# daooshee/ReReVST-Code

Hardware: AMD Instinct MI355X
Metric: stylized frames/sec at 512x512, 1 style (higher is better)
Workload: dtype f32

## Files before the change

include/rerevst_hip.h:

```cpp
#ifndef REREVST_HIP_H
#define REREVST_HIP_H

#include <stddef.h>
#include <stdint.h>

#ifdef __cplusplus
extern "C" {
#endif

typedef struct rrv_ctx* rrv_handle;

enum {
    RRV_OK = 0,
    RRV_E_ARG = -1,
    RRV_E_HIP = -2,
    RRV_E_WEIGHTS = -3,
    RRV_E_STATE = -4,
    RRV_E_NOMEM = -5,
    RRV_E_DEBUG = -6,
    RRV_E_COMM = -7
};

#define RRV_STATE_FLOATS 17536
#define RRV_MAX_STYLES 8
// ... 157 lines not shown
int rrv_set_yuv16_matrix(rrv_handle h, const float m[12]);
int rrv_set_yuv16_input_matrix(rrv_handle h, const float n[12]);

int rrv_prepare_style_image_device(rrv_handle h, const void* d_style, rrv_image_desc in, int Hs, int Ws, int style_id, void* hip_stream);
int rrv_add_image_device(rrv_handle h, const void* d_frame, rrv_image_desc in, int H, int W, void* hip_stream);

int rrv_get_preclamp(rrv_handle h, float* out, int H, int W);
int rrv_get_preclamp_image(rrv_handle h, float* out, int H, int W, int b);

int rrv_sync(rrv_handle h);

int rrv_set_pipeline(rrv_handle h, int n_slots);

int rrv_set_grid_share(rrv_handle h, int share);

int rrv_set_host_io(rrv_handle h, int mode);

int rrv_debug_copy_tensor(rrv_handle h, int slot, int index, int H, int W, float* host, size_t cap, size_t* floats);

int rrv_debug_copy_tensor_ex(rrv_handle h, int slot, int index, int image, int H, int W, float* host, size_t cap, size_t* floats,
                             int* layout, int* channels);

#define RRV_DBG_STATE_SET 0
#define RRV_DBG_STYLE_PRED 1
int rrv_debug_copy_state(rrv_handle h, int what, int slot, int image, float* out, int n);

int rrv_set_caller_stream(rrv_handle h, void* hip_stream, int enable);

int rrv_host_alloc(size_t bytes, void** out);
int rrv_host_free(void* p);
// ... 18 lines not shown
```

rerevst-code_amd/_lib.py:

```python
import ctypes as C
import os

HERE = os.path.dirname(os.path.abspath(__file__))
LIB_PATH = os.environ.get("RRV_LIB_PATH") or os.path.join(HERE, "librerevst_hip.so")
STATE_FLOATS = 17536
MAX_STYLES = 8

_lib = None


class ImageDesc(C.Structure):
    _fields_ = [("dtype", C.c_int), ("layout", C.c_int), ("space", C.c_int)]


DT_U8, DT_F32 = 0, 1
DT_U16 = 2
LAY_HWC_BGR, LAY_CHW_RGB = 0, 1
LAY_I420, LAY_NV12 = 2, 3
LAY_I420_16, LAY_P016 = 8, 9
YUV_BT601, YUV_BT709 = 0, 1
SP_PIXEL, SP_UNIT, SP_NORM = 0, 1, 2
TF_PAD_CROP, TF_FRAME_MODE, TF_ON_STREAM, TF_WEIGHTS_DEVICE = 1, 2, 4, 8
DBG_STATE_SET, DBG_STYLE_PRED = 0, 1

# ... 74 lines not shown
    "rrv_yuv_input_matrix_depth": (C.c_int, [C.c_int, C.c_int, C.c_int, C.POINTER(C.c_float)]),
    "rrv_set_yuv16_matrix": (C.c_int, [C.c_void_p, C.POINTER(C.c_float)]),
    "rrv_set_yuv16_input_matrix": (C.c_int, [C.c_void_p, C.POINTER(C.c_float)]),
    "rrv_prepare_style_image_device": (C.c_int, [C.c_void_p, C.c_void_p, ImageDesc, C.c_int, C.c_int, C.c_int, C.c_void_p]),
    "rrv_add_image_device": (C.c_int, [C.c_void_p, C.c_void_p, ImageDesc, C.c_int, C.c_int, C.c_void_p]),
    "rrv_get_preclamp": (C.c_int, [C.c_void_p, C.c_void_p, C.c_int, C.c_int]),
    "rrv_get_preclamp_image": (C.c_int, [C.c_void_p, C.c_void_p, C.c_int, C.c_int, C.c_int]),
    "rrv_sync": (C.c_int, [C.c_void_p]),
    "rrv_set_pipeline": (C.c_int, [C.c_void_p, C.c_int]),
    "rrv_set_host_io": (C.c_int, [C.c_void_p, C.c_int]),
    "rrv_debug_copy_tensor": (C.c_int, [C.c_void_p, C.c_int, C.c_int, C.c_int, C.c_int, C.c_void_p, C.c_size_t, C.POINTER(C.c_size_t)]),
    "rrv_debug_copy_tensor_ex": (C.c_int, [C.c_void_p, C.c_int, C.c_int, C.c_int, C.c_int, C.c_int, C.c_void_p, C.c_size_t,
                                           C.POINTER(C.c_size_t), C.POINTER(C.c_int), C.POINTER(C.c_int)]),
    "rrv_debug_copy_state": (C.c_int, [C.c_void_p, C.c_int, C.c_int, C.c_int, C.c_void_p, C.c_int]),
    "rrv_set_grid_share": (C.c_int, [C.c_void_p, C.c_int]),
    "rrv_set_caller_stream": (C.c_int, [C.c_void_p, C.c_void_p, C.c_int]),
    "rrv_host_alloc": (C.c_int, [C.c_size_t, C.POINTER(C.c_void_p)]),
    "rrv_host_free": (C.c_int, [C.c_void_p]),
    "rrv_host_register": (C.c_int, [C.c_void_p, C.c_size_t]),
    "rrv_host_unregister": (C.c_int, [C.c_void_p]),
    "rrv_set_debug": (C.c_int, [C.c_void_p, C.c_int]),
    "rrv_debug_selftest": (C.c_int, [C.c_void_p]),
    "rrv_debug_fail_alloc": (C.c_int, [C.c_void_p, C.c_int]),
    "rrv_profile_begin": (C.c_int, [C.c_void_p]),
    "rrv_profile_end": (C.c_int, [C.c_void_p]),
    "rrv_profile_count": (C.c_int, [C.c_void_p]),
    "rrv_profile_entry": (C.c_int, [C.c_void_p, C.c_int, C.POINTER(C.c_char_p), C.POINTER(C.c_float),
                                    C.POINTER(C.c_double), C.POINTER(C.c_double), C.POINTER(C.c_double)]),
}

# ... 41 lines not shown
```

rerevst-code_amd/build.py:

```python
import os
import subprocess
import sys

HERE = os.path.dirname(os.path.abspath(__file__))
CSRC = os.path.join(HERE, "csrc")
LIB = os.path.join(HERE, "librerevst_hip.so")
SOURCES = ["rerevst_hip.hip"]
HEADERS = ["conv_mfma.h", "conv_wino.h", "conv_ups5.h", "conv_wino_split.h", "conv_f43.h", "conv_thin.h", "prep_kernels.h", "mask_kernels.h", "../../include/rerevst_hip.h"]


def _stale():
    if not os.path.exists(LIB):
        return True
    t = os.path.getmtime(LIB)
    return any(os.path.getmtime(os.path.join(CSRC, f)) > t for f in SOURCES + HEADERS)


def build_lib(force=False, verbose=True, extra=()):
    if not force and not _stale():
        return LIB
    hipcc = os.environ.get("HIPCC", "/opt/rocm/bin/hipcc")
    cmd = [hipcc, "--offload-arch=gfx950", "-O3", "-std=c++17", "-shared", "-fPIC",
           "-Wno-unused-result", *extra,
           *[os.path.join(CSRC, s) for s in SOURCES], "-o", LIB]
# ... 9 lines not shown
```

rerevst-code_amd/csrc/conv_mfma.h:

```cpp
#pragma once
#include <hip/hip_runtime.h>
#include <stdint.h>

typedef float f32x16 __attribute__((ext_vector_type(16)));
typedef float f32x4 __attribute__((ext_vector_type(4)));

enum {
    E_RELU = 1,
    E_LRELU = 2,
    E_NORM1 = 4,
    E_RES = 8,
    E_RES_UPS = 16,
    E_NORM2 = 32,
    E_POOL = 64
};

struct ConvP {
    const float* in;
    int Hi, Wi, Cin;
    float* out;
    int H, W, Cout;
    int B;
    int in_bstride0;
    const float* wpk;
    const float* bias;
    const float* n1;
    const float* res;
    int Hr, Wr;
    const float* n2;
    const float* sty;
    int tiles_x, tiles_y;
    int xcd_slabs;
    float* sc_out;
    int ty0, tx0;
    long long* dbg;
    int cstride;
    int cin_slab_step;
    int par_bstride, bias_bstride;
    long long w_bstride;
    int out_p8;
};

template <int BN>
struct WaveCfg {
    static constexpr int WAVES_N = (BN >= 64) ? 2 : 1;
    static constexpr int WAVES_M = 4 / WAVES_N;
    static constexpr int WN_SUB = BN / 32 / WAVES_N;
    static constexpr int WM_SUB = 4 / WAVES_M;
};

__device__ __forceinline__ void glds16(const float* src, char* lds_wave_base) {
    __builtin_amdgcn_global_load_lds((const __attribute__((address_space(1))) void*)src,
                                     (__attribute__((address_space(3))) void*)lds_wave_base, 16, 0, 0);
}
// ... 244 lines not shown
```

rerevst-code_amd/csrc/rerevst_hip.hip:

```cpp
#include <hip/hip_runtime.h>
#include <dlfcn.h>
#include <stddef.h>
#include <stdint.h>
#include <string.h>
#include <algorithm>
#include <cmath>
#include <thread>
#include <stdio.h>
#include <map>
#include <condition_variable>
#include <mutex>
#include <string>
#include <vector>

#include "../../include/rerevst_hip.h"
#include "conv_mfma.h"
#include "conv_wino.h"
#include "conv_wino_split.h"
#include "conv_f43.h"
#include "conv_thin.h"
#include "prep_kernels.h"
#include "mask_kernels.h"

namespace {

const int NORM_CH[11] = {512, 512, 256, 128, 64, 256, 256, 128, 128, 64, 64};
enum { N_DEC0 = 0, N_DEC1, N_DEC2, N_DEC3, N_DEC4, N_S4N1, N_S4N2, N_S3N1, N_S3N2, N_S2N1, N_S2N2 };
const int STYLE_CH[4] = {64, 128, 256, 512};
struct StateLayout {
    int norm[11], filt[6], sty[4];
    StateLayout() {
        int o = 0;
        for (int i = 0; i < 11; ++i) { norm[i] = o; o += 4 * NORM_CH[i]; }
// ... 162 lines not shown
    PrepPlan prep;
    uint8_t* pend_u8 = nullptr; size_t pend_cap = 0; int pend_n = 0;
    InFmt pend_in = IN_BGR8;
    static constexpr int BLEND_W_RING = 4, BLEND_W_FLOATS = 64 * RRV_MAX_STYLES;
    struct BlendW { float* dev = nullptr; float* pin = nullptr; hipEvent_t ev[BLEND_W_RING] = {nullptr}; bool used[BLEND_W_RING] = {false}; unsigned gen = 0; } blend_w[2];
    const float* last_pre = nullptr; int last_pre_H = 0, last_pre_W = 0, last_pre_B = 0;
    struct StageBufs { uint8_t* in = nullptr; void* out = nullptr; size_t in_cap = 0, out_cap = 0; };
    struct HostStage {
        StageBufs dev, pin; hipEvent_t in_done = nullptr, k_done = nullptr, out_done = nullptr;
        float *mask = nullptr, *mask_pin = nullptr; size_t mask_cap = 0, mask_pin_cap = 0;
    } hstage[4];
    hipStream_t copy_in = nullptr, copy_out = nullptr;
    struct Ticket { long id = -1; void* out = nullptr; size_t out_bytes = 0; bool open = false; } tickets[4];
    long next_ticket = 0;
    int grid_share = 1;
    int f43_mode = 1;
    unsigned f43_layers = F43_DEFAULT_LAYERS;
    bool illcond = false;
    bool enc_p8_tables = false;
    int p8 = 3;
    bool f43_path = false;
    unsigned direct_layers = 0;
    int ms_group = 0;
    YuvSide yuv_in, yuv_out;
    int host_io = 0;
    int n_cus = 256;
    int debug = 0;
    int fail_alloc_in = 0;
    bool profiling = false;
    std::vector<ProfEntry> prof;
// ... 182 lines not shown
    return RRV_OK;
}

struct ConvCall {
    const Tens* in; Tens* out; const ConvW* w;
    int H, W;
    bool ups = false; int epi = 0;
    Tens* sc_out = nullptr;
    int wy0 = 0, wx0 = 0, wy1 = 0, wx1 = 0;
    const float* n1 = nullptr; const Tens* res = nullptr; const float* n2 = nullptr; const float* sty = nullptr;
    int B = 1;
    int ksplit = 0;
    const float* bias = nullptr;
    int par_bstride = 0, bias_bstride = 0; long long w_bstride = 0;
    bool direct = false;
    bool in_p8 = false, out_p8 = false;
};

template <int BN, int TAPS, int EPI>
void conv_launch(const ConvP& p, dim3 grid, hipStream_t s) {
    hipLaunchKernelGGL((conv_mfma_k<BN, TAPS, EPI>), grid, dim3(256), 0, s, p);
}

typedef void (*ConvFn)(const ConvP&, dim3, hipStream_t);
typedef hipError_t (*AttrFn)();
struct ConvKey { int BN, TAPS, UPS, EPI; ConvFn fn; const char* name; AttrFn attr; ConvFn fn_img = nullptr; };
#define CK(BN, TAPS, UPS, EPI) {BN, TAPS, UPS, EPI, &conv_launch<BN, TAPS, EPI>, "conv_mfma<" #BN "," #TAPS "," #EPI ">", nullptr}
const ConvKey CONV_TABLE[] = {
    CK(128, 1, 0, 0), CK(64, 1, 0, 0),
    CK(32, 9, 0, 0),
// ... 11 lines not shown
}
template <int EPI, int NW, int UPS, int SC, int PERIMG = 0>
hipError_t wino_attr() {
    hipError_t e = hipFuncSetAttribute((const void*)conv_wino_k<EPI, 0, NW, UPS, SC, 0>, hipFuncAttributeMaxDynamicSharedMemorySize, wino_smem<NW, UPS, SC>());
    if (e == hipSuccess && PERIMG) e = hipFuncSetAttribute((const void*)conv_wino_k<EPI, 0, NW, UPS, SC, 1>, hipFuncAttributeMaxDynamicSharedMemorySize, wino_smem<NW, UPS, SC>());
    return e;
}
template <int EPI, int PERIMG>
void wsplit_launch(const ConvP& p, dim3 grid, hipStream_t s) {
    hipLaunchKernelGGL((conv_wino_split_k<EPI, PERIMG>), grid, dim3(512), WSPLIT_SMEM_BYTES, s, p);
}
template <int EPI, int PERIMG>
hipError_t wsplit_attr() {
    hipError_t e = hipFuncSetAttribute((const void*)conv_wino_split_k<EPI, 0>, hipFuncAttributeMaxDynamicSharedMemorySize, WSPLIT_SMEM_BYTES);
    if (e == hipSuccess && PERIMG) e = hipFuncSetAttribute((const void*)conv_wino_split_k<EPI, 1>, hipFuncAttributeMaxDynamicSharedMemorySize, WSPLIT_SMEM_BYTES);
    return e;
}
template <int EPI, int LAY = 0>
void f43_launch(const ConvP& p, dim3 grid, hipStream_t s) {
    hipLaunchKernelGGL((conv_f43_k<EPI, LAY>), grid, dim3(F43Geo::NT), F43Geo::SMEM, s, p);
}
template <int EPI, int LAY = 0>
hipError_t f43_attr() { return hipFuncSetAttribute((const void*)conv_f43_k<EPI, LAY>, hipFuncAttributeMaxDynamicSharedMemorySize, F43Geo::SMEM); }
#define FK(EPI) {32, 9, 0, EPI, &f43_launch<EPI>, "conv_f43<" #EPI ">", &f43_attr<EPI>, nullptr}
struct F43LayKey { int EPI, LAY; ConvFn fn; const char* name; AttrFn attr; };
#define FKL(EPI, LAY) {EPI, LAY, &f43_launch<EPI, LAY>, "conv_f43<" #EPI ", " #LAY ">", &f43_attr<EPI, LAY>}
#define WK(EPI) {32, 9, 0, EPI, &wsplit_launch<EPI, 0>, "conv_wino<" #EPI ">", &wsplit_attr<EPI, 0>, nullptr}
#define WKI(EPI) {32, 9, 0, EPI, &wsplit_launch<EPI, 0>, "conv_wino<" #EPI ">", &wsplit_attr<EPI, 1>, &wsplit_launch<EPI, 1>}
#define UW(EPI) {32, 9, 1, EPI, &wino_launch<EPI, UPW_NW, 1, 0>, "conv_upw<" #EPI ">", &wino_attr<EPI, UPW_NW, 1, 0>}
#define UWS(EPI) {32, 29, 1, EPI, &wino_launch<EPI, UPW_NW, 1, 1>, "conv_upw_sc<" #EPI ">", &wino_attr<EPI, UPW_NW, 1, 1>}
#define UWSI(EPI) {32, 29, 1, EPI, &wino_launch<EPI, UPW_NW, 1, 1>, "conv_upw_sc<" #EPI ">", &wino_attr<EPI, UPW_NW, 1, 1, 1>, &wino_launch<EPI, UPW_NW, 1, 1, 1>}
const ConvKey WINO_TABLE[] = {
    WK(E_RELU), WK(E_RELU | E_POOL), WKI(E_RELU | E_NORM1) , WKI(E_LRELU | E_NORM1 | E_RES_UPS | E_NORM2), WKI(E_LRELU),
    WKI(0),
    WKI(E_RES), WKI(E_RES | E_NORM2),
    UW(E_LRELU | E_NORM1), UW(E_LRELU),
    UWSI(E_LRELU | E_NORM1),
    UWS(E_LRELU),
};

const ConvKey F43_TABLE[] = { FK(E_RELU), FK(E_RELU | E_POOL), FK(E_RELU | E_NORM1), FK(E_LRELU | E_NORM1 | E_RES_UPS | E_NORM2) };
const F43LayKey F43_LAY_TABLE[] = {
    FKL(E_RELU | E_POOL, 3), FKL(E_RELU, 3),
    FKL(E_RELU | E_POOL, 1),
    FKL(E_LRELU | E_NORM1 | E_RES_UPS | E_NORM2, 1),
};

unsigned resident_wgs(rrv_handle h, int occ) {
    unsigned r = (unsigned)h->n_cus * (unsigned)occ;
    if (h->grid_share > 1) {
        r = (r / h->grid_share) & ~7u;
        if (r < 8) r = 8;
    }
    return r;
}
// ... 19 lines not shown
    const ConvKey* k = nullptr;
    bool wino = false;
    bool f43 = !c.direct && use_f43(h, w, c.B, c.H, c.W, c.epi, c.ups, c.ksplit, c.bias_bstride != 0 || c.w_bstride != 0) &&
               !((c.wy0 | c.wx0 | c.wy1 | c.wx1) & 31);
    if (f43) {
        f43 = false;
        for (const ConvKey& e : F43_TABLE)
            if (e.EPI == c.epi) { k = &e; f43 = true; wino = true; break; }
    }
    const bool fuse_sc = c.ups && c.sc_out != nullptr;
    if (fuse_sc && !w.pk_ups_sc) return fail(h, RRV_E_ARG, "conv: no shortcut-fused pack for this layer");
    if (!f43 && !c.direct && (c.ups ? w.pk_ups != nullptr : w.pk_wino != nullptr)) {
        for (const ConvKey& e : WINO_TABLE)
            if (e.EPI == c.epi && e.UPS == (int)c.ups && (e.TAPS == 29) == fuse_sc) { k = &e; wino = true; break; }
    }
    const int ks = c.ksplit > 1 ? c.ksplit : 1;
    if (ks > 1 && !(wino && !c.ups && w.Cout == 32 && (w.Cin % (32 * ks)) == 0 && c.bias))
        return fail(h, RRV_E_ARG, "conv: split K needs the row-split kernel, a 32-cout layer, an even number of 16-channel chunks per slice and a split bias");
    if (!k && !c.ups) {
        for (const ConvKey& e : CONV_TABLE)
            if (e.BN == w.BN && e.TAPS == w.taps && e.EPI == c.epi) { k = &e; break; }
    }
    if (!k) {
        char b[128];
        snprintf(b, sizeof b, "no conv kernel for BN=%d taps=%d ups=%d epi=%d", w.BN, w.taps, (int)c.ups, c.epi);
        return fail(h, RRV_E_ARG, b);
    }
    const int lay = (c.in_p8 ? 1 : 0) | (c.out_p8 ? 2 : 0);
    ConvFn lay_fn = nullptr;
    const char* lay_name = nullptr;
// ... 10 lines not shown
    p.in_bstride0 = 1;
    p.wpk = f43 ? w.pk_f43 : wino ? (c.ups ? (fuse_sc ? w.pk_ups_sc : w.pk_ups) : w.pk_wino) : w.pk; p.bias = w.bias;
    if (fuse_sc) {
        if (c.sc_out->H != c.in->H || c.sc_out->W != c.in->W || c.sc_out->C != w.Cout) return fail(h, RRV_E_ARG, "conv: shortcut output geometry mismatch");
        p.sc_out = c.sc_out->p;
    }
    if (!p.wpk) return fail(h, RRV_E_ARG, "conv: weights not packed for this kernel"); p.n1 = c.n1; p.n2 = c.n2; p.sty = c.sty;
    if (c.bias) p.bias = c.bias;
    p.par_bstride = c.par_bstride; p.bias_bstride = c.bias_bstride; p.w_bstride = c.w_bstride;
    if (ups_p8) { if (!wino) return fail(h, RRV_E_ARG, "conv: no upsample-fused kernel for this layer"); p.out_p8 = 1; }
    if ((c.par_bstride | c.bias_bstride || c.w_bstride) && !wino) return fail(h, RRV_E_ARG, "conv: per-image state needs a transform-domain kernel");
    if (c.ups && (c.bias_bstride || c.w_bstride)) return fail(h, RRV_E_ARG, "conv: the upsample-fused kernel shares weights and bias over the images of a launch");
    if (ks > 1) {
        p.Cin = w.Cin / ks; p.cstride = w.Cin; p.cin_slab_step = w.Cin / ks; p.Cout = 32 * ks;
    }
    if (c.res) { p.res = c.res->p; p.Hr = c.res->H; p.Wr = c.res->W; }
    p.tiles_x = (c.W + 15) / 16; p.tiles_y = (c.H + 7) / 8;
    if ((c.in_p8 ? c.in->C != 8 || c.in->B < c.B * (w.Cin / 8) : c.in->C != w.Cin) ||
        (c.out_p8 ? c.out->C != 8 || c.out->B < c.B * (w.Cout / 8) : c.out->C != w.Cout * ks)) return fail(h, RRV_E_ARG, "conv: channel mismatch");
    const int eh = c.ups ? c.H / 2 : c.H, ew = c.ups ? c.W / 2 : c.W;
    if (c.in->H != eh || c.in->W != ew + (c.in_p8 ? 6 : 0)) return fail(h, RRV_E_ARG, "conv: input geometry mismatch");
    const int oh = (c.epi & E_POOL) ? c.H / 2 : c.H, ow = (c.epi & E_POOL) ? c.W / 2 : c.W;
    if (c.out->H != oh || c.out->W != ow + (c.out_p8 ? 6 : 0)) return fail(h, RRV_E_ARG, "conv: output geometry mismatch");
    const int TS = f43 || fuse_sc ? 32 : 16;
    if (wino) { p.tiles_x = (c.W + TS - 1) / TS; p.tiles_y = (c.H + TS - 1) / TS; }
    double win_frac = 1.0;
    if (wino && c.wy1 > c.wy0 && c.wx1 > c.wx0) {
        if ((c.wy0 | c.wx0 | c.wy1 | c.wx1) & 15) return fail(h, RRV_E_ARG, "conv: window must be tile aligned");
        int wy0 = c.wy0, wx0 = c.wx0, wy1 = c.wy1, wx1 = c.wx1;
        if (TS == 32 && !f43) {
            wy0 &= ~31; wx0 &= ~31; wy1 = (wy1 + 31) & ~31; wx1 = (wx1 + 31) & ~31;
            if (wy1 > ((c.H + 31) & ~31)) wy1 = (c.H + 31) & ~31;
            if (wx1 > ((c.W + 31) & ~31)) wx1 = (c.W + 31) & ~31;
        }
        p.ty0 = wy0 / TS; p.tx0 = wx0 / TS;
        p.tiles_y = (wy1 - wy0) / TS; p.tiles_x = (wx1 - wx0) / TS;
        const int TD = fuse_sc ? 32 : 16;
        win_frac = ((double)(wy1 - wy0) * (wx1 - wx0)) / ((double)((c.H + TD - 1) / TD * TD) * ((c.W + TD - 1) / TD * TD));
    }
    dim3 grid((unsigned)(p.tiles_x * p.tiles_y * c.B), (unsigned)(w.Cout / w.BN));
    if (wino) {
        const unsigned slabs = (unsigned)(w.Cout / 32) * ks;
        const unsigned items = (unsigned)(p.tiles_x * p.tiles_y * c.B) * slabs;
        const unsigned resident = resident_wgs(h, fuse_sc ? Ups5Geo::OCC : c.ups ? WinoGeo<UPW_NW, 1>::OCC : 1);
        grid = dim3(items < resident ? items : resident, 1);
        p.xcd_slabs = (grid.x % 8 == 0 && (grid.x / 8) % slabs == 0) ? 1 : 0;
    }
    const double px = (double)c.B * c.H * c.W * win_frac;
    const double cin = w.Cin;
    const double flops_sc = fuse_sc ? 2.0 * c.B * c.in->H * c.in->W * (double)w.Cout * cin : 0.0;
    const double flops = 2.0 * px * w.Cout * cin * w.taps + flops_sc;
    const double flops_exec = 2.0 * px * w.Cout * cin * (f43 ? 2.25 : wino ? (c.ups ? (fuse_sc ? 29.0 / 16.0 : 2.25) : 4.0) : (double)w.taps);
    const double bytes = 4.0 * ((double)c.B * c.in->H * c.in->W * cin + (double)c.B * oh * ow * w.Cout +
                                (c.res ? (double)c.B * c.res->H * c.res->W * w.Cout : 0.0) + (double)w.Cout * cin * w.taps +
                                (fuse_sc ? (double)c.B * c.in->H * c.in->W * w.Cout + (double)w.Cout * cin : 0.0));
    hipStream_t s = h->stream;
    ConvFn fn = lay_fn ? lay_fn : k->fn;
    if (wino && !f43 && (c.par_bstride | c.bias_bstride || c.w_bstride)) {
        if (!k->fn_img) return fail(h, RRV_E_ARG, "conv: this layer has no per-image-state kernel");
        fn = k->fn_img;
    }
    stamp(h, c.out, c.B);
    if (fuse_sc) stamp(h, c.sc_out, c.B);
    if (h->profiling) {
        char nm[160];
        snprintf(nm, sizeof nm, "%s@%dx%d@%dx%d", lay_name ? lay_name : k->name, w.Cin, w.Cout, c.H, c.W);
        return launch(h, nm, flops, bytes, [&] { fn(p, grid, s); }, flops_exec);
    }
    return launch(h, lay_name ? lay_name : k->name, flops, bytes, [&] { fn(p, grid, s); }, flops_exec);
// ... 387 lines not shown
    d.B = B; d.H = H; d.W = W;
    return RRV_OK;
}

int filter_down(rrv_handle h, const Tens* cur, DecPlan& d, int f, int B) {
    const int split = kf_split(cur->H, cur->W);
    if (split == 1) {
        ConvCall c{cur, &d.d, &h->cur->fold_down[f], cur->H, cur->W}; c.B = B; c.epi = E_LRELU;
        if (h->state_images) { c.w_bstride = 32 * 512 * 16; c.bias_bstride = 256; }
        return conv(h, c);
    }
    Tens& t = d.dpart;
    ConvCall c{cur, &t, &h->cur->fold_down[f], cur->H, cur->W}; c.B = B; c.epi = 0; c.ksplit = split; c.bias = h->cur->fold_down[f].bias;
    if (h->state_images) { c.w_bstride = 32 * 512 * 16; c.bias_bstride = 256; }
    RCHK(conv(h, c));
    const long npix = (long)B * (d.d.H + 2) * (d.d.W + 2);
    stamp(h, &d.d, B);
    return launch(h, "sum_parts", 0, 4.0 * 32 * (split + 1) * npix, [&] {
        const long nb = (npix * 8 + 255) / 256;
        hipLaunchKernelGGL(sum_parts_lrelu_k, dim3((unsigned)(nb < 4096 ? nb : 4096)), dim3(256), 0, h->stream, (const float*)t.p, d.d.p, split, npix);
    });
}

int filter_up(rrv_handle h, const Tens* cur, DecPlan& d, Tens* out, int f, int B) {
    const float* st = h->cur->active;
    ConvCall u{&d.d, out, &h->cur->fold_up[f], cur->H, cur->W}; u.B = B;
    if (h->state_images) { u.w_bstride = 512 * 32 * 16; u.par_bstride = RRV_STATE_FLOATS; }
    u.epi = E_RES | (f == 2 ? E_NORM2 : 0); u.res = cur;
    if (f == 2) { u.n2 = st + SL.norm[N_DEC1]; u.sty = st + SL.sty[3]; }
    return conv(h, u);
}

struct Win { int y0, x0, y1, x1; };

struct BlkDesc { const char* name; int cout, n1, n2, nada, sty; };
const BlkDesc BLKS[3] = {{"slice4", 256, N_S4N1, N_S4N2, N_DEC2, 2}, {"slice3", 128, N_S3N1, N_S3N2, N_DEC3, 1}, {"slice2", 64, N_S2N1, N_S2N2, N_DEC4, 0}};

int resblock_frame(rrv_handle h, int B, int k, const Tens& in, DecPlan& d, const Win* wa = nullptr, const Win* wo = nullptr) {
    const BlkDesc& b = BLKS[k];
    Tens &xs = d.xs[k], &a = d.a[k], &o = d.o[k], &qa = d.qa[k];
    const float* st = h->cur->active;
// ... 556 lines not shown
    h->dev = device;
    (void)rrv_yuv_input_matrix(RRV_YUV_BT601, 0, h->yuv_in.m8);
    (void)rrv_yuv_matrix(RRV_YUV_BT601, 0, h->yuv_out.m8);
    bool ok = hipSetDevice(device) == hipSuccess;
    for (int i = 0; ok && i < RRV_MAX_SLOTS; ++i) ok = hipStreamCreateWithFlags(&h->streams[i], hipStreamNonBlocking) == hipSuccess;
    if (!ok) {
        delete h;
        return RRV_E_HIP;
    }
    h->stream = h->streams[0];
    ok = ok && hipStreamCreateWithFlags(&h->copy_in, hipStreamNonBlocking) == hipSuccess && hipStreamCreateWithFlags(&h->copy_out, hipStreamNonBlocking) == hipSuccess;
    for (int i = 0; ok && i < RRV_MAX_SLOTS; ++i) ok = hipEventCreateWithFlags(&h->slot_ev[i], hipEventDisableTiming) == hipSuccess;
    for (auto& st : h->hstage)
        for (hipEvent_t* e : {&st.in_done, &st.k_done, &st.out_done}) ok = ok && hipEventCreateWithFlags(e, hipEventDisableTiming) == hipSuccess;
    for (const ConvKey& e : WINO_TABLE)
        if (ok && e.attr) ok = e.attr() == hipSuccess;
    for (const ConvKey& e : F43_TABLE)
        if (ok && e.attr) ok = e.attr() == hipSuccess;
    for (const F43LayKey& e : F43_LAY_TABLE)
        if (ok && e.attr) ok = e.attr() == hipSuccess;
    if (!ok) {
        delete h;
        return RRV_E_HIP;
    }
    {
        hipDeviceProp_t prop;
        if (hipGetDeviceProperties(&prop, device) == hipSuccess && prop.multiProcessorCount > 0) h->n_cus = prop.multiProcessorCount;
        const int masked = cu_mask_count(getenv("HSA_CU_MASK"), device, h->n_cus);
        if (masked > 0 && masked < h->n_cus) h->n_cus = masked;
        if (const char* e = getenv("RRV_CUS")) { const int n = atoi(e); if (n >= 1 && n <= 1024) h->n_cus = n; }
// ... 1568 lines not shown
int rrv_sync(rrv_handle h) {
    if (!h) return RRV_E_ARG;
    HIPCHK(hipSetDevice(h->dev));
    return sync_all(h);
}

int rrv_set_pipeline(rrv_handle h, int n_slots) {
    if (!h || n_slots < 1 || n_slots > RRV_MAX_SLOTS) return RRV_E_ARG;
    HIPCHK(hipSetDevice(h->dev));
    RCHK(sync_all(h));
    h->n_slots = n_slots;
    h->next_slot = 0;
    return RRV_OK;
}

int rrv_set_grid_share(rrv_handle h, int share) {
    if (!h || share < 1 || share > 4) return RRV_E_ARG;
    h->grid_share = share;
    return RRV_OK;
}

int rrv_set_f43(rrv_handle h, int mode) {
    if (!h || mode < 0 || mode > 2) return RRV_E_ARG;
    RCHK(sync_all(h));
    h->f43_mode = mode;
    return RRV_OK;
}

int rrv_set_multistyle_group(rrv_handle h, int frames) {
    if (!h || frames < 0 || frames > rrv_ctx::MS_GROUP_MAX) return RRV_E_ARG;
// ... 159 lines not shown
```

rerevst-code_amd/framework.py:

```python
import collections
import ctypes as C

import numpy as np

from . import _lib
from .video import YUV_FORMATS, YUV_FORMAT_NAMES, YUV_STANDARDS, _yuv_depth, yuv_frame_bytes
from .weights import weight_table, load_checkpoint


class RRVError(RuntimeError):
    pass


def pinned_empty(shape, dtype=np.float32):
    import weakref
    lib = _lib.load()
    dt = np.dtype(dtype)
    n = int(np.prod(shape)) * dt.itemsize
    ptr = C.c_void_p()
    if lib.rrv_host_alloc(max(n, 1), C.byref(ptr)) != 0:
        raise MemoryError("rrv_host_alloc(%d) failed" % n)
    buf = (C.c_char * max(n, 1)).from_address(ptr.value)
    weakref.finalize(buf, lib.rrv_host_free, ptr)
    return np.frombuffer(buf, dtype=dt, count=int(np.prod(shape))).reshape(shape)
# ... 597 lines not shown
                    a.out_desc, flags | (_lib.TF_WEIGHTS_DEVICE if wd is not None else 0), stream))
                continue
            self._chk(plain_fn(self._h, C.c_void_p(xb[b0].data_ptr()), a.in_desc, nb, a.H, a.W,
                               C.c_void_p(ob[b0].data_ptr()), a.out_desc, flags, stream))
        return out

    def sync(self):
        self._chk(self._lib.rrv_sync(self._h))

    def set_caller_stream(self, stream_ptr, enable=True):
        self._chk(self._lib.rrv_set_caller_stream(self._h, C.c_void_p(stream_ptr), 1 if enable else 0))

    def set_f43(self, mode):
        self._chk(self._lib.rrv_set_f43(self._h, int(mode)))

    def set_grid_share(self, share):
        self._chk(self._lib.rrv_set_grid_share(self._h, int(share)))

    def debug_tensor(self, slot, index, H, W):
        n = C.c_size_t(0)
        self._chk(self._lib.rrv_debug_copy_tensor(self._h, int(slot), int(index), int(H), int(W), None, 0, C.byref(n)))
        out = np.empty(n.value, np.float32)
        self._chk(self._lib.rrv_debug_copy_tensor(self._h, int(slot), int(index), int(H), int(W), out.ctypes.data_as(C.c_void_p), n.value, C.byref(n)))
        return out

    def debug_tensor_ex(self, slot, index, H, W, image=0):
        n, lay, ch = C.c_size_t(0), C.c_int(0), C.c_int(0)
        args = (self._h, int(slot), int(index), int(image), int(H), int(W))
        self._chk(self._lib.rrv_debug_copy_tensor_ex(*args, None, 0, C.byref(n), C.byref(lay), C.byref(ch)))
        out = np.empty(n.value, np.float32)
# ... 149 lines not shown
```

Before: 836.2.

## Fuse split-K partial sum and LeakyReLU into KernelFilter up-conv Winograd kernel

Adds a dedicated Winograd up-convolution kernel for the 32-channel KernelFilter path that reads the split-K partial-sum tensor directly, sums the parts and applies LeakyReLU while staging input tiles into LDS. This removes the separate sum_parts_lrelu kernel launch and its write and re-read of the summed tensor. The kernel also walks a contiguous span of (tile, output-slab) units per workgroup, so an input tile is transformed once and reused across output slabs. The cost is reading the wider partial-sum input inside the conv, plus a more complex kernel with hand-placed waits and barriers.

```diff
diff --git a/include/rerevst_hip.h b/include/rerevst_hip.h
--- a/include/rerevst_hip.h
+++ b/include/rerevst_hip.h
@@ -195,6 +195,8 @@
 
 int rrv_set_grid_share(rrv_handle h, int share);
 
+int rrv_set_kf_up(rrv_handle h, int mode);
+
 int rrv_set_host_io(rrv_handle h, int mode);
 
 int rrv_debug_copy_tensor(rrv_handle h, int slot, int index, int H, int W, float* host, size_t cap, size_t* floats);
diff --git a/rerevst-code_amd/_lib.py b/rerevst-code_amd/_lib.py
--- a/rerevst-code_amd/_lib.py
+++ b/rerevst-code_amd/_lib.py
@@ -112,6 +112,7 @@
                                            C.POINTER(C.c_size_t), C.POINTER(C.c_int), C.POINTER(C.c_int)]),
     "rrv_debug_copy_state": (C.c_int, [C.c_void_p, C.c_int, C.c_int, C.c_int, C.c_void_p, C.c_int]),
     "rrv_set_grid_share": (C.c_int, [C.c_void_p, C.c_int]),
+    "rrv_set_kf_up": (C.c_int, [C.c_void_p, C.c_int]),
     "rrv_set_caller_stream": (C.c_int, [C.c_void_p, C.c_void_p, C.c_int]),
     "rrv_host_alloc": (C.c_int, [C.c_size_t, C.POINTER(C.c_void_p)]),
     "rrv_host_free": (C.c_int, [C.c_void_p]),
diff --git a/rerevst-code_amd/build.py b/rerevst-code_amd/build.py
--- a/rerevst-code_amd/build.py
+++ b/rerevst-code_amd/build.py
@@ -6,7 +6,7 @@
 CSRC = os.path.join(HERE, "csrc")
 LIB = os.path.join(HERE, "librerevst_hip.so")
 SOURCES = ["rerevst_hip.hip"]
-HEADERS = ["conv_mfma.h", "conv_wino.h", "conv_ups5.h", "conv_wino_split.h", "conv_f43.h", "conv_thin.h", "prep_kernels.h", "mask_kernels.h", "../../include/rerevst_hip.h"]
+HEADERS = ["conv_mfma.h", "conv_wino.h", "conv_ups5.h", "conv_wino_split.h", "conv_wino_up32.h", "conv_f43.h", "conv_thin.h", "prep_kernels.h", "mask_kernels.h", "../../include/rerevst_hip.h"]
 
 
 def _stale():
diff --git a/rerevst-code_amd/csrc/conv_mfma.h b/rerevst-code_amd/csrc/conv_mfma.h
--- a/rerevst-code_amd/csrc/conv_mfma.h
+++ b/rerevst-code_amd/csrc/conv_mfma.h
@@ -38,6 +38,8 @@
     int cin_slab_step;
     int par_bstride, bias_bstride;
     long long w_bstride;
+    int in_parts;
+    int slab_span;
     int out_p8;
 };
 
diff --git a/rerevst-code_amd/csrc/conv_wino_up32.h b/rerevst-code_amd/csrc/conv_wino_up32.h
--- /dev/null
+++ b/rerevst-code_amd/csrc/conv_wino_up32.h
@@ -0,0 +1,262 @@
+#pragma once
+#include "conv_wino_split.h"
+
+#ifndef WUP32_ABL
+#define WUP32_ABL 0
+#endif
+#define WUP32_STAGE_GROUP 3
+
+#define WUP32_SMEM_BYTES (WSPLIT_SMEM_BYTES + WINO_PAR_BYTES)
+
+template <int EPI, int PERIMG = 0>
+__global__ __launch_bounds__(512, 1) void conv_wino_up32_k(const ConvP p) {
+    static_assert((EPI & ~(E_RES | E_NORM2)) == 0 && (EPI & E_RES), "the KernelFilter up-convolution: residual, optional second normalisation");
+    using G = WinoGeo<8, 0>;
+    constexpr int RAW_BYTES = G::RAW_BYTES, U_BYTES = G::U_BYTES, U_LDS = G::U_LDS, NT = G::NT;
+    static_assert(G::U_IT == 4, "U block = 4 LDS-DMA instructions per thread");
+    extern __shared__ __attribute__((aligned(16))) char smem[];
+    const int tid = threadIdx.x;
+    const int wave = __builtin_amdgcn_readfirstlane(tid >> 6);
+    const int lane = tid & 63, t = lane & 15, q = lane >> 4;
+    const int tr = t >> 3, tc = t & 7;
+    const int tg = wave >> 1;
+    const int half = wave & 1;
+    const float sgn = half ? -1.f : 1.f;
+    const int cs = p.cstride;
+    const int n_ntiles = p.Cout >> 5;
+
+    const int n_units = p.tiles_x * p.tiles_y * p.B * n_ntiles;
+    int unit = blockIdx.x * p.slab_span;
+    const int unit_end = min(unit + p.slab_span, n_units);
+    struct Item { int tx, ty, b, s0, s1; };
+    auto item_at = [&](int u) {
+        Item r;
+        const int pix = u / n_ntiles;
+        r.s0 = u - pix * n_ntiles;
+        r.s1 = min(n_ntiles, r.s0 + unit_end - u);
+        r.tx = pix % p.tiles_x; r.ty = (pix / p.tiles_x) % p.tiles_y; r.b = pix / (p.tiles_x * p.tiles_y);
+        return r;
+    };
+    auto in_of = [&](const Item& a) {
+        return p.in + (size_t)a.b * (size_t)(p.Hi + 2) * (p.Wi + 2) * cs + (size_t)(((a.ty + p.ty0) * 16) * (p.Wi + 2) + (a.tx + p.tx0) * 16) * cs;
+    };
+    auto w_of = [&](const Item& a) { return p.wpk + (size_t)a.s0 * (2 * 16 * 32 * 16) + (PERIMG ? (size_t)a.b * p.w_bstride : (size_t)0); };
+
+    char* const par = smem + 2 * RAW_BYTES + 2 * U_LDS;
+    char* const xch = par + 2 * WINO_PAR_BYTES;
+    auto stage_params = [&](int ntile, int img) {
+        if (wave < 2) {
+            const int e = tid;
+            const int row = e >> 3, col = (e & 7) * 4;
+            const float* src = p.bias;
+            const int pb = PERIMG ? img * p.par_bstride : 0;
+            int off = ntile * 32 + col + (PERIMG ? img * p.bias_bstride : 0);
+            if (row >= 5 && row <= 8) { src = (EPI & E_NORM2) ? p.n2 : p.bias; off = (EPI & E_NORM2) ? ntile * 32 + col + pb + (row - 5) * p.Cout : off; }
+            if (row >= 9) { src = (EPI & E_NORM2) ? p.sty : p.bias; off = (EPI & E_NORM2) ? ntile * 32 + col + pb + (row - 9) * p.Cout : off; }
+            if (row > 10) { src = p.bias; off = ntile * 32 + (PERIMG ? img * p.bias_bstride : 0); }
+            glds16(src + off, par + (ntile & 1) * WINO_PAR_BYTES + wave * 1024);
+        }
+    };
+
+    constexpr int N_PIECE = 324 * 8, N_ROWS = (N_PIECE + NT - 1) / NT;
+    struct Piece { int src, dst; };
+    auto piece_at = [&](int row) {
+        const int e = row * NT + tid;
+        const bool ok = e < N_PIECE;
+        const int P = ok ? e >> 3 : 0, cq = ok ? e & 7 : 0;
+        const int hf = P >= G::HALF, rem = P - hf * G::HALF;
+        const int hy = rem / 9, hx = 2 * (rem - hy * 9) + hf;
+        return Piece{(hy * (p.Wi + 2) + hx) * cs + 4 * cq, ok ? (cq >> 2) * RAW_BYTES + P * 64 + (((cq & 3) ^ ((hx >> 1) & 3)) << 4) : -1};
+    };
+    auto piece_load = [&](const float* in_t, const Piece pc, auto& part) {
+        constexpr int PARTS = sizeof(part) / sizeof(part[0]);
+#pragma unroll
+        for (int k = 0; k < PARTS; ++k) part[k] = *(const f32x4*)(in_t + pc.src + 32 * k);
+    };
+    auto piece_store = [&](const Piece pc, const auto& part) {
+        constexpr int PARTS = sizeof(part) / sizeof(part[0]);
+        f32x4 o = part[0];
+#pragma unroll
+        for (int k = 1; k < PARTS; ++k) o += part[k];
+        if (PARTS > 1) {
+#pragma unroll
+            for (int c = 0; c < 4; ++c) o[c] = o[c] >= 0.f ? o[c] : o[c] * 0.2f;
+        }
+        if (pc.dst >= 0) *(f32x4*)(smem + pc.dst) = o;
+    };
+
+    const unsigned lds0 = (unsigned)(size_t)(__attribute__((address_space(3))) char*)smem;
+    const unsigned offU = lds0 + 2 * RAW_BYTES + t * 64 + ((q ^ ((0 - (t >> 2)) & 3)) << 4);
+    const unsigned ubA = offU + (half ? 12 : 0) * 2048;
+    const unsigned ubB = offU + (half ? 8 : 4) * 2048;
+
+    f32x4 acc[8][2];
+    f32x4 va[8], vb[8];
+    auto transform = [&](int chunk, f32x4 (&v)[8]) {
+        f32x4 d[12];
+#pragma unroll
+        for (int dx = 0; dx < 4; ++dx)
+#pragma unroll
+            for (int b = 0; b < 3; ++b) {
+                const int hy = 4 * tg + 2 * tr + (half ? 3 - b : b), hx = 2 * tc + dx;
+                const int P = (hx & 1) * G::HALF + hy * 9 + (hx >> 1);
+                d[dx * 3 + b] = *(const f32x4*)(smem + chunk * RAW_BYTES + P * 64 + ((q ^ ((hx >> 1) & 3)) << 4));
+            }
+#pragma unroll
+        for (int dx = 0; dx < 4; ++dx) {
+            v[dx * 2 + 0] = f4sub(d[dx * 3 + 0], d[dx * 3 + 2]);
+            v[dx * 2 + 1] = f4fma(d[dx * 3 + 2], sgn, d[dx * 3 + 1]);
+        }
+#pragma unroll
+        for (int rl = 0; rl < 2; ++rl) {
+            const f32x4 e0 = v[0 + rl], e1 = v[2 + rl], e2 = v[4 + rl], e3 = v[6 + rl];
+            v[0 + rl] = f4sub(e0, e2); v[2 + rl] = f4add(e1, e2); v[4 + rl] = f4sub(e2, e1); v[6 + rl] = f4sub(e1, e3);
+        }
+    };
+
+    auto chunk_body = [&](auto par_c, const f32x4 (&vcur)[8], const rsrc_t rs_u, const int usoff, auto&& hook) {
+        constexpr int PAR = decltype(par_c)::value;
+        constexpr bool FIRST = PAR == 0;
+        char* const udst = smem + 2 * RAW_BYTES + (1 - PAR) * U_LDS;
+        constexpr int UI = PAR * U_LDS;
+        f32x4 u[4][2];
+        u[0][0] = lds_rd128<UI + 0>(ubA); u[0][1] = lds_rd128<UI + 1024>(ubA);
+        u[1][0] = lds_rd128<UI + 2048>(ubA); u[1][1] = lds_rd128<UI + 2048 + 1024>(ubA);
+        static_for([&](auto ic) {
+            constexpr int i = decltype(ic)::value;
+            if constexpr (i + 2 < 8) {
+                constexpr int n = i + 2, k = n & 3;
+                u[n & 3][0] = lds_rd128<UI + k * 2048>(n < 4 ? ubA : ubB);
+                u[n & 3][1] = lds_rd128<UI + k * 2048 + 1024>(n < 4 ? ubA : ubB);
+            }
+            lds_release2<(i + 1 < 8 ? 2 : 0) + (i + 2 < 8 ? 2 : 0)>(u[i & 3][0], u[i & 3][1]);
+            __builtin_amdgcn_sched_barrier(0);
+            if constexpr (i < G::U_IT) bufld16_rs(rs_u, udst + (i * NT + wave * 64) * 16, tid * 16, usoff + i * NT * 16);
+            const f32x4 vv = vcur[(i & 3) * 2 + (i >> 2)];
+#pragma unroll
+            for (int s = 0; s < 4; ++s)
+#pragma unroll
+                for (int nb = 0; nb < 2; ++nb)
+                    acc[i][nb] = __builtin_amdgcn_mfma_f32_16x16x4f32(u[i & 3][nb][s], vv[s], (FIRST && s == 0) ? f32x4{0.f, 0.f, 0.f, 0.f} : acc[i][nb], 0, 0, 0);
+            hook(ic);
+        }, std::make_integer_sequence<int, 8>{});
+    };
+    auto no_hook = [](auto) {};
+
+    auto run = [&](auto parts_c) {
+        constexpr int PARTS = decltype(parts_c)::value;
+        Item cur{};
+        bool have = unit < unit_end;
+        const float* w_t = p.wpk;
+        const float* in_t = p.in;
+        if (have) {
+            cur = item_at(unit);
+            w_t = w_of(cur);
+            in_t = in_of(cur);
+#pragma unroll
+            for (int it = 0; it < G::U_IT; ++it) bufld16(w_t, smem + 2 * RAW_BYTES + (it * NT + wave * 64) * 16, tid * 16, it * NT * 16);
+        }
+        while (have) {
+            if (!(WUP32_ABL & 1) || unit == (int)blockIdx.x * p.slab_span) {
+                for (int g = 0; g < N_ROWS; g += WUP32_STAGE_GROUP) {
+                    f32x4 part[WUP32_STAGE_GROUP][PARTS];
+#pragma unroll
+                    for (int j = 0; j < WUP32_STAGE_GROUP; ++j) if (g + j < N_ROWS) piece_load(in_t, piece_at(g + j), part[j]);
+#pragma unroll
+                    for (int j = 0; j < WUP32_STAGE_GROUP; ++j) if (g + j < N_ROWS) piece_store(piece_at(g + j), part[j]);
+                }
+            }
+            __syncthreads();
+            transform(0, va);
+            transform(1, vb);
+            const int e_y0 = (cur.ty + p.ty0) * 16, e_x0 = (cur.tx + p.tx0) * 16, e_b = cur.b;
+            const int n_slabs = cur.s1 - cur.s0;
+            unit += n_slabs;
+            const bool have_nxt = unit < unit_end;
+            Item nxt = cur;
+            if (have_nxt) nxt = item_at(unit);
+            const float* w_n = have_nxt ? w_of(nxt) : w_t;
+            const float* in_n = have_nxt ? in_of(nxt) : in_t;
+            const rsrc_t rs_t = make_rsrc(w_t), rs_n = make_rsrc(w_n);
+            const float* res_b = p.res + (size_t)e_b * (size_t)(p.Hr + 2) * (p.Wr + 2) * p.Cout;
+            const int yb = e_y0 + 4 * tg + 2 * tr, xb = e_x0 + 2 * tc;
+            const int y = yb + half;
+            int rpix[2];
+#pragma unroll
+            for (int j = 0; j < 2; ++j) rpix[j] = (y < p.H && xb + j < p.W) ? ((y + 1) * (p.Wr + 2) + xb + j + 1) * p.Cout : 0;
+
+            const rsrc_t rs_out = make_rsrc(p.out + (size_t)e_b * (size_t)(p.H + 2) * (p.W + 2) * p.Cout);
+            constexpr unsigned NO_PIXEL = 0x80000000u;
+            unsigned pend_off[2] = {NO_PIXEL, NO_PIXEL};
+            int pend_par = 0;
+            f32x4 Tc[2][2];
+            f32x4 resv[2][2];
+            const char* const theirs = xch + (wave ^ 1) * 4096 + lane * 16;
+            auto epi_step = [&](auto ic) {
+                constexpr int nb = decltype(ic)::value >> 1, j = decltype(ic)::value & 1;
+                const char* pl = par + pend_par * WINO_PAR_BYTES + (nb * 16 + 4 * q) * 4;
+                const f32x4 bias = *(const f32x4*)(pl);
+                const f32x4 rc = *(const f32x4*)(theirs + (j * 2 + nb) * 1024);
+                const f32x4 Y = e4add(Tc[j][nb], rc);
+                f32x4 o = e4add(Y, bias);
+                o = e4add(o, resv[nb][j]);
+                if (EPI & E_NORM2) {
+                    const f32x4 m2 = *(const f32x4*)(pl + 640), r2 = *(const f32x4*)(pl + 768), lo2 = *(const f32x4*)(pl + 896), hi2 = *(const f32x4*)(pl + 1024);
+                    const f32x4 smean = *(const f32x4*)(pl + 1152), sstd = *(const f32x4*)(pl + 1280);
+                    o = e4fma(f4norm_clamp(o, m2, r2, lo2, hi2), sstd, smean);
+                }
+#if defined(__HIP_DEVICE_COMPILE__)
+                typedef unsigned u32x4 __attribute__((ext_vector_type(4)));
+                if constexpr (!(WUP32_ABL & 2)) __builtin_amdgcn_raw_buffer_store_b128(__builtin_bit_cast(u32x4, o), rs_out, (int)(pend_off[j] + nb * 64), 0, 0);
+#endif
+            };
+            constexpr int N_ST = (WUP32_ABL & 2) ? 0 : 1;
+
+            for (int r = 0; r < n_slabs; ++r) {
+                const int e_ntile = cur.s0 + r;
+                stage_params(e_ntile, e_b);
+                auto hook0 = [&](auto ic) {
+                    if constexpr (decltype(ic)::value < 4) epi_step(ic);
+                    if constexpr (decltype(ic)::value == 4) {
+#pragma unroll
+                        for (int nb = 0; nb < 2; ++nb)
+#pragma unroll
+                            for (int j = 0; j < 2; ++j) resv[nb][j] = *(const f32x4*)(res_b + rpix[j] + e_ntile * 32 + 4 * q + nb * 16);
+                    }
+                };
+                const bool last = r + 1 == n_slabs;
+                chunk_body(std::integral_constant<int, 0>{}, va, rs_t, (2 * r + 1) * U_BYTES, hook0);
+                if constexpr (!(WUP32_ABL & 4)) asm volatile("s_waitcnt vmcnt(%0) lgkmcnt(0)\n\ts_barrier" :: "n"(4 + N_ST) : "memory");
+                chunk_body(std::integral_constant<int, 1>{}, vb, last ? rs_n : rs_t, last ? 0 : (2 * r + 2) * U_BYTES, no_hook);
+                asm volatile("s_nop 15\n\ts_nop 15\n\ts_nop 15" : "+v"(acc[0][0]), "+v"(acc[0][1]), "+v"(acc[1][0]), "+v"(acc[1][1]), "+v"(acc[2][0]), "+v"(acc[2][1]), "+v"(acc[3][0]), "+v"(acc[3][1]), "+v"(acc[4][0]), "+v"(acc[4][1]), "+v"(acc[5][0]), "+v"(acc[5][1]), "+v"(acc[6][0]), "+v"(acc[6][1]), "+v"(acc[7][0]), "+v"(acc[7][1]));
+                char* mine = xch + wave * 4096 + lane * 16;
+#pragma unroll
+                for (int nb = 0; nb < 2; ++nb) {
+                    f32x4 T[2][2];
+#pragma unroll
+                    for (int rl = 0; rl < 2; ++rl) {
+                        T[rl][0] = e4add(e4add(acc[rl * 4 + 0][nb], acc[rl * 4 + 1][nb]), acc[rl * 4 + 2][nb]);
+                        T[rl][1] = f4sub(f4sub(acc[rl * 4 + 1][nb], acc[rl * 4 + 2][nb]), acc[rl * 4 + 3][nb]);
+                    }
+#pragma unroll
+                    for (int j = 0; j < 2; ++j) {
+                        *(f32x4*)(mine + (j * 2 + nb) * 1024) = T[1][j];
+                        Tc[j][nb] = f4fma(T[1][j], sgn, T[0][j]);
+                    }
+                }
+                if constexpr (!(WUP32_ABL & 4)) __syncthreads();
+#pragma unroll
+                for (int j = 0; j < 2; ++j)
+                    pend_off[j] = (y < p.H && xb + j < p.W) ? (unsigned)((((y + 1) * (p.W + 2) + xb + j + 1) * p.Cout + e_ntile * 32 + 4 * q) * 4) : NO_PIXEL;
+                pend_par = e_ntile & 1;
+            }
+            static_for([&](auto ic) { epi_step(ic); }, std::make_integer_sequence<int, 4>{});
+            cur = nxt; have = have_nxt; w_t = w_n; in_t = in_n;
+        }
+    };
+    if (p.in_parts == 8) run(std::integral_constant<int, 8>{});
+    else if (p.in_parts == 4) run(std::integral_constant<int, 4>{});
+    else if (p.in_parts == 2) run(std::integral_constant<int, 2>{});
+    else run(std::integral_constant<int, 1>{});
+    asm volatile("s_waitcnt vmcnt(0)" ::: "memory");
+}
diff --git a/rerevst-code_amd/csrc/rerevst_hip.hip b/rerevst-code_amd/csrc/rerevst_hip.hip
--- a/rerevst-code_amd/csrc/rerevst_hip.hip
+++ b/rerevst-code_amd/csrc/rerevst_hip.hip
@@ -17,6 +17,7 @@
 #include "conv_mfma.h"
 #include "conv_wino.h"
 #include "conv_wino_split.h"
+#include "conv_wino_up32.h"
 #include "conv_f43.h"
 #include "conv_thin.h"
 #include "prep_kernels.h"
@@ -209,6 +210,7 @@
     struct Ticket { long id = -1; void* out = nullptr; size_t out_bytes = 0; bool open = false; } tickets[4];
     long next_ticket = 0;
     int grid_share = 1;
+    int kf_up = 1;
     int f43_mode = 1;
     unsigned f43_layers = F43_DEFAULT_LAYERS;
     bool illcond = false;
@@ -421,6 +423,7 @@
     const float* bias = nullptr;
     int par_bstride = 0, bias_bstride = 0; long long w_bstride = 0;
     bool direct = false;
+    int in_parts = 0;
     bool in_p8 = false, out_p8 = false;
 };
 
@@ -462,6 +465,16 @@
 hipError_t wsplit_attr() {
     hipError_t e = hipFuncSetAttribute((const void*)conv_wino_split_k<EPI, 0>, hipFuncAttributeMaxDynamicSharedMemorySize, WSPLIT_SMEM_BYTES);
     if (e == hipSuccess && PERIMG) e = hipFuncSetAttribute((const void*)conv_wino_split_k<EPI, 1>, hipFuncAttributeMaxDynamicSharedMemorySize, WSPLIT_SMEM_BYTES);
+    return e;
+}
+template <int EPI, int PERIMG>
+void wup32_launch(const ConvP& p, dim3 grid, hipStream_t s) {
+    hipLaunchKernelGGL((conv_wino_up32_k<EPI, PERIMG>), grid, dim3(512), WUP32_SMEM_BYTES, s, p);
+}
+template <int EPI>
+hipError_t wup32_attr() {
+    hipError_t e = hipFuncSetAttribute((const void*)conv_wino_up32_k<EPI, 0>, hipFuncAttributeMaxDynamicSharedMemorySize, WUP32_SMEM_BYTES);
+    if (e == hipSuccess) e = hipFuncSetAttribute((const void*)conv_wino_up32_k<EPI, 1>, hipFuncAttributeMaxDynamicSharedMemorySize, WUP32_SMEM_BYTES);
     return e;
 }
 template <int EPI, int LAY = 0>
@@ -487,6 +500,9 @@
     UWS(E_LRELU),
 };
 
+#define WU(EPI) {32, 9, 0, EPI, &wup32_launch<EPI, 0>, "conv_wino_up32<" #EPI ">", &wup32_attr<EPI>, &wup32_launch<EPI, 1>}
+const ConvKey UP32_TABLE[] = { WU(E_RES), WU(E_RES | E_NORM2) };
+
 const ConvKey F43_TABLE[] = { FK(E_RELU), FK(E_RELU | E_POOL), FK(E_RELU | E_NORM1), FK(E_LRELU | E_NORM1 | E_RES_UPS | E_NORM2) };
 const F43LayKey F43_LAY_TABLE[] = {
     FKL(E_RELU | E_POOL, 3), FKL(E_RELU, 3),
@@ -536,6 +552,12 @@
         for (const ConvKey& e : WINO_TABLE)
             if (e.EPI == c.epi && e.UPS == (int)c.ups && (e.TAPS == 29) == fuse_sc) { k = &e; wino = true; break; }
     }
+    bool up32 = false;
+    if (wino && !f43 && !c.ups && w.Cin == 32 && h->kf_up)
+        for (const ConvKey& e : UP32_TABLE)
+            if (e.EPI == c.epi) { k = &e; up32 = true; break; }
+    if (c.in_parts > 1 && !(up32 && (c.in_parts == 2 || c.in_parts == 4 || c.in_parts == 8)))
+        return fail(h, RRV_E_ARG, "conv: a partial-sum input needs the transform-once kernel and 2, 4 or 8 parts");
     const int ks = c.ksplit > 1 ? c.ksplit : 1;
     if (ks > 1 && !(wino && !c.ups && w.Cout == 32 && (w.Cin % (32 * ks)) == 0 && c.bias))
         return fail(h, RRV_E_ARG, "conv: split K needs the row-split kernel, a 32-cout layer, an even number of 16-channel chunks per slice and a split bias");
@@ -576,9 +598,11 @@
     if (ks > 1) {
         p.Cin = w.Cin / ks; p.cstride = w.Cin; p.cin_slab_step = w.Cin / ks; p.Cout = 32 * ks;
     }
+    const int in_parts = c.in_parts > 1 ? c.in_parts : 1;
+    if (up32) { p.in_parts = c.in_parts; p.cstride = w.Cin * in_parts; }
     if (c.res) { p.res = c.res->p; p.Hr = c.res->H; p.Wr = c.res->W; }
     p.tiles_x = (c.W + 15) / 16; p.tiles_y = (c.H + 7) / 8;
-    if ((c.in_p8 ? c.in->C != 8 || c.in->B < c.B * (w.Cin / 8) : c.in->C != w.Cin) ||
+    if ((c.in_p8 ? c.in->C != 8 || c.in->B < c.B * (w.Cin / 8) : c.in->C != w.Cin * in_parts) ||
         (c.out_p8 ? c.out->C != 8 || c.out->B < c.B * (w.Cout / 8) : c.out->C != w.Cout * ks)) return fail(h, RRV_E_ARG, "conv: channel mismatch");
     const int eh = c.ups ? c.H / 2 : c.H, ew = c.ups ? c.W / 2 : c.W;
     if (c.in->H != eh || c.in->W != ew + (c.in_p8 ? 6 : 0)) return fail(h, RRV_E_ARG, "conv: input geometry mismatch");
@@ -607,6 +631,11 @@
         const unsigned resident = resident_wgs(h, fuse_sc ? Ups5Geo::OCC : c.ups ? WinoGeo<UPW_NW, 1>::OCC : 1);
         grid = dim3(items < resident ? items : resident, 1);
         p.xcd_slabs = (grid.x % 8 == 0 && (grid.x / 8) % slabs == 0) ? 1 : 0;
+        if (up32) {
+            static const unsigned forced = [] { const char* e = getenv("RRV_KF_SPAN"); const int v = e ? atoi(e) : 0; return (v == 16 || v == 8 || v == 4) ? (unsigned)v : 0u; }();
+            p.slab_span = (int)(forced ? forced : (items + resident - 1) / resident);
+            grid = dim3((items + p.slab_span - 1) / p.slab_span, 1);
+        }
     }
     const double px = (double)c.B * c.H * c.W * win_frac;
     const double cin = w.Cin;
@@ -615,6 +644,7 @@
     const double flops_exec = 2.0 * px * w.Cout * cin * (f43 ? 2.25 : wino ? (c.ups ? (fuse_sc ? 29.0 / 16.0 : 2.25) : 4.0) : (double)w.taps);
     const double bytes = 4.0 * ((double)c.B * c.in->H * c.in->W * cin + (double)c.B * oh * ow * w.Cout +
                                 (c.res ? (double)c.B * c.res->H * c.res->W * w.Cout : 0.0) + (double)w.Cout * cin * w.taps +
+                                (in_parts - 1) * (double)c.B * c.in->H * c.in->W * cin +
                                 (fuse_sc ? (double)c.B * c.in->H * c.in->W * w.Cout + (double)w.Cout * cin : 0.0));
     hipStream_t s = h->stream;
     ConvFn fn = lay_fn ? lay_fn : k->fn;
@@ -1032,9 +1062,10 @@
     ConvCall c{cur, &t, &h->cur->fold_down[f], cur->H, cur->W}; c.B = B; c.epi = 0; c.ksplit = split; c.bias = h->cur->fold_down[f].bias;
     if (h->state_images) { c.w_bstride = 32 * 512 * 16; c.bias_bstride = 256; }
     RCHK(conv(h, c));
+    if (h->kf_up && !h->profiling) return RRV_OK;
     const long npix = (long)B * (d.d.H + 2) * (d.d.W + 2);
     stamp(h, &d.d, B);
-    return launch(h, "sum_parts", 0, 4.0 * 32 * (split + 1) * npix, [&] {
+    return launch(h, h->kf_up ? "sum_parts_tap" : "sum_parts", 0, 4.0 * 32 * (split + 1) * npix, [&] {
         const long nb = (npix * 8 + 255) / 256;
         hipLaunchKernelGGL(sum_parts_lrelu_k, dim3((unsigned)(nb < 4096 ? nb : 4096)), dim3(256), 0, h->stream, (const float*)t.p, d.d.p, split, npix);
     });
@@ -1042,7 +1073,10 @@
 
 int filter_up(rrv_handle h, const Tens* cur, DecPlan& d, Tens* out, int f, int B) {
     const float* st = h->cur->active;
-    ConvCall u{&d.d, out, &h->cur->fold_up[f], cur->H, cur->W}; u.B = B;
+    const int split = kf_split(cur->H, cur->W);
+    const bool parts = h->kf_up && split > 1;
+    ConvCall u{parts ? &d.dpart : &d.d, out, &h->cur->fold_up[f], cur->H, cur->W}; u.B = B;
+    if (parts) u.in_parts = split;
     if (h->state_images) { u.w_bstride = 512 * 32 * 16; u.par_bstride = RRV_STATE_FLOATS; }
     u.epi = E_RES | (f == 2 ? E_NORM2 : 0); u.res = cur;
     if (f == 2) { u.n2 = st + SL.norm[N_DEC1]; u.sty = st + SL.sty[3]; }
@@ -1629,6 +1663,8 @@
     for (auto& st : h->hstage)
         for (hipEvent_t* e : {&st.in_done, &st.k_done, &st.out_done}) ok = ok && hipEventCreateWithFlags(e, hipEventDisableTiming) == hipSuccess;
     for (const ConvKey& e : WINO_TABLE)
+        if (ok && e.attr) ok = e.attr() == hipSuccess;
+    for (const ConvKey& e : UP32_TABLE)
         if (ok && e.attr) ok = e.attr() == hipSuccess;
     for (const ConvKey& e : F43_TABLE)
         if (ok && e.attr) ok = e.attr() == hipSuccess;
@@ -3227,6 +3263,12 @@
     return RRV_OK;
 }
 
+int rrv_set_kf_up(rrv_handle h, int mode) {
+    if (!h || mode < 0 || mode > 1) return RRV_E_ARG;
+    h->kf_up = mode;
+    return RRV_OK;
+}
+
 int rrv_set_grid_share(rrv_handle h, int share) {
     if (!h || share < 1 || share > 4) return RRV_E_ARG;
     h->grid_share = share;
diff --git a/rerevst-code_amd/framework.py b/rerevst-code_amd/framework.py
--- a/rerevst-code_amd/framework.py
+++ b/rerevst-code_amd/framework.py
@@ -635,6 +635,9 @@
     def set_f43(self, mode):
         self._chk(self._lib.rrv_set_f43(self._h, int(mode)))
 
+    def set_kf_up(self, mode):
+        self._chk(self._lib.rrv_set_kf_up(self._h, int(mode)))
+
     def set_grid_share(self, share):
         self._chk(self._lib.rrv_set_grid_share(self._h, int(share)))
 
```

New measurement: 836.1. No clear change (-0.0%).
